# NeuralRevenant/semantic-query-engine

Measured on AMD Instinct MI355X. Metric: k-NN queries/sec (brute-force cosine top-10, 1024-d, 10M vectors), higher is better.
Workload: dtype i8; 1 GPU; flat cosine top-10, N=10000000 x 1024 fp32 (int8 collect scan (per-row-scaled int8 copy, sample-derived thresholds) + fp32 re-score of the candidates, exactness certified per query, bf16 collect pass for uncertified queries), batch=1024 queries/step, index row-sharded over 1 GPU(s); rows=10000000, dim=1024, batch=1024, k=10, parallelism=shard1, scan_mode=int8

## Files before the change

### include/sqe.h

```cpp
#ifndef SQE_H
#define SQE_H

#include <stdint.h>

#ifdef __cplusplus
extern "C" {
#endif

#define SQE_VERSION 100

typedef struct sqe_ctx sqe_ctx;
typedef struct sqe_index sqe_index;
typedef struct sqe_cache sqe_cache;
typedef struct sqe_encoder sqe_encoder;
typedef struct sqe_tokenizer sqe_tokenizer;

enum {
    SQE_OK = 0,
    SQE_ERR_INVALID = -1,
    SQE_ERR_HIP = -2,
    SQE_ERR_OOM = -3,
    SQE_ERR_STATE = -4,
    SQE_ERR_UNSUPPORTED = -5,
    SQE_ERR_IO = -6
// ... 57 lines not shown
int sqe_index_search_collapsed_device(sqe_index* idx, const float* q_dev, int B, int k,
                                      float* cos_out_dev, int64_t* id_out_dev, int64_t* key_out_dev);

int sqe_index_train(sqe_index* idx, const float* x_host, int64_t n, int iters, uint64_t seed);
int sqe_index_train_device(sqe_index* idx, const float* x_dev, int64_t n, int iters, uint64_t seed);
int sqe_index_ivf_export(sqe_index* idx, float* centroids_host, int32_t* assign_host);

typedef struct sqe_i8_launch_t {
    int64_t rows;
    int64_t tile_stride;
    int32_t dim, B, b_pad, k;
    int32_t tile_rows;
    int32_t q_pitch;
    int32_t query_block;
    int32_t n_chunks;
    int32_t list_cap;
    int32_t sample_int8;
    int32_t sample_step;
    int32_t sample_tiles, sample_chunks, sample_b_pad, sample_m;
    int32_t uncertified;
    int32_t pool_cap;
} sqe_i8_launch_t;
enum { SQE_I8_ROWS = 0, SQE_I8_ROW_SCALES = 1, SQE_I8_QUERIES = 2, SQE_I8_THRESHOLDS = 3, SQE_I8_LIST_COUNTS = 4, SQE_I8_LISTS = 5,
       SQE_I8_SAMPLE_BEST = 6, SQE_I8_POOL_COUNTS = 7, SQE_I8_POOLS = 8, SQE_I8_QUERIES_TILED = 9 };
int sqe_index_i8_last(sqe_index* idx, sqe_i8_launch_t* out);
int sqe_index_i8_read(sqe_index* idx, int what, int64_t offset, void* out_host, int64_t bytes);

typedef struct sqe_index_state_t {
    int64_t rows;
    int64_t i8_rows;
    int64_t i8_tile_stride;
    int32_t dim;
    int32_t scan_pitch;
    int32_t last_B;
    int32_t last_i8;
} sqe_index_state_t;
enum { SQE_STATE_SCAN_BF16 = 0, SQE_STATE_RESID_MAX = 1, SQE_STATE_I8_RESID_MAX = 2, SQE_STATE_QN = 3, SQE_STATE_Q_RESID = 4,
       SQE_STATE_Q8_RESID = 5, SQE_STATE_Q8_SCALES = 6 };
int sqe_index_state(sqe_index* idx, sqe_index_state_t* out);
int sqe_index_state_read(sqe_index* idx, int what, int64_t offset, void* out_host, int64_t bytes);

int sqe_index_save(sqe_index* idx, const char* path);
int sqe_index_load(sqe_ctx* ctx, const char* path, sqe_index** out);

int sqe_merge_topk_device(sqe_ctx* ctx, const float* cos_parts_dev, const int64_t* id_parts_dev,
                          int64_t part_stride_bytes, int P, int B, int k,
                          float* cos_out_dev, int64_t* id_out_dev);
// ... 67 lines not shown
```

### semantic_query_engine_amd/csrc/api.hip

```cpp
#include <math.h>
#include <stdio.h>
#include <stdlib.h>
#include <string.h>

#include <algorithm>
#include <memory>
#include <new>
#include <vector>

#include "internal.h"

namespace sqe {

static thread_local std::string g_last_error;

void set_error(const std::string& msg) { g_last_error = msg; }
int fail(int code, const std::string& msg) {
    g_last_error = msg;
    return code;
}

int index_grow(sqe_index* idx, int64_t need_rows, hipStream_t s) {
    if (need_rows <= idx->cap) return SQE_OK;
    const int64_t n = idx->n.load();
// ... 395 lines not shown

int sqe_index_i8_read(sqe_index* idx, int what, int64_t offset, void* out_host, int64_t bytes) {
    if (!idx || (!out_host && bytes > 0)) return fail(SQE_ERR_INVALID, "sqe_index_i8_read: null argument");
    if (idx->group || idx->ivf) return fail(SQE_ERR_UNSUPPORTED, "sqe_index_i8_read: single-device FLAT indexes only");
    OpScope op(idx->ctx, idx->ord, true);
    const sqe_i8_launch_t& L = idx->i8_launch;
    const bool copy_only = what == SQE_I8_ROWS || what == SQE_I8_ROW_SCALES;
    if (L.rows == 0 && !(copy_only && idx->i8db.p && idx->i8_rows > 0))
        return fail(SQE_ERR_STATE, copy_only ? "sqe_index_i8_read: this index has no int8 copy of its rows"
                                             : "sqe_index_i8_read: this index has not answered a search with the int8 first pass");
    const int64_t tiles = L.rows ? (L.rows + L.tile_rows - 1) / L.tile_rows : (idx->i8_rows + SCAN_BM - 1) / SCAN_BM;
    const void* src = nullptr;
    int64_t size = 0;
    switch (what) {
        case SQE_I8_ROWS: src = idx->i8db.p; size = tiles * idx->i8_tile_stride; break;
        case SQE_I8_ROW_SCALES: src = idx->i8sxi.p; size = tiles * SCAN_BM * 4; break;
        case SQE_I8_QUERIES: src = idx->q8.p; size = (int64_t)L.b_pad * L.q_pitch; break;
        case SQE_I8_QUERIES_TILED: src = idx->q8t.p; size = ((int64_t)L.b_pad + 255) / 256 * 256 * L.dim; break;
        case SQE_I8_THRESHOLDS: src = idx->i8thr_int.p; size = (int64_t)L.b_pad * 4; break;
        case SQE_I8_LIST_COUNTS: src = idx->cand_cnt.p; size = (int64_t)L.n_chunks * L.b_pad * 4; break;
        case SQE_I8_LISTS: src = idx->cand.p; size = (int64_t)L.n_chunks * L.b_pad * L.list_cap * 8; break;
        case SQE_I8_POOL_COUNTS: src = idx->i8ovf_cnt.p; size = (int64_t)L.b_pad * 4; break;
        case SQE_I8_POOLS: src = idx->i8ovf.p; size = (int64_t)L.b_pad * L.pool_cap * 8; break;
        case SQE_I8_SAMPLE_BEST:
            if (!L.sample_int8) return fail(SQE_ERR_STATE, "sqe_index_i8_read: the threshold pass of the last search did not run in int8");
            src = idx->i8samp.p; size = (int64_t)L.sample_chunks * L.sample_b_pad * 16 * 8; break;
        default: return fail(SQE_ERR_INVALID, "sqe_index_i8_read: unknown buffer");
    }
    if (offset < 0 || bytes < 0 || offset + bytes > size) return fail(SQE_ERR_INVALID, "sqe_index_i8_read: range outside the buffer");
    if (bytes == 0) return SQE_OK;
    SQE_HIP(hipMemcpyAsync(out_host, static_cast<const char*>(src) + offset, (size_t)bytes, hipMemcpyDeviceToHost, op.s));
    SQE_HIP(hipStreamSynchronize(op.s));
    return SQE_OK;
}

int sqe_index_state(sqe_index* idx, sqe_index_state_t* out) {
    if (!idx || !out) return fail(SQE_ERR_INVALID, "sqe_index_state: null argument");
    if (idx->group || idx->ivf) return fail(SQE_ERR_UNSUPPORTED, "sqe_index_state: single-device FLAT indexes only");
    OpScope op(idx->ctx, idx->ord, true);
    out->rows = idx->n.load();
    out->i8_rows = idx->i8db.p ? idx->i8_rows : 0;
    out->i8_tile_stride = idx->i8db.p ? idx->i8_tile_stride : 0;
    out->dim = idx->dim;
    out->scan_pitch = idx->pitch;
    out->last_B = idx->last_B;
    out->last_i8 = idx->last_i8 ? 1 : 0;
// ... 500 lines not shown
```

### semantic_query_engine_amd/csrc/internal.h

```cpp
#pragma once

#include <atomic>
#include <mutex>
#include <string>
#include <vector>

#include "kernels.h"

namespace sqe {

struct DevBuf {
    void* p = nullptr;
    size_t bytes = 0;
    DevBuf() = default;
    DevBuf(const DevBuf&) = delete;
    DevBuf& operator=(const DevBuf&) = delete;
    ~DevBuf() { release(); }
    void release() {
        if (p) (void)hipFree(p);
        p = nullptr;
        bytes = 0;
    }
    int ensure(size_t need) {
        if (need <= bytes) return SQE_OK;
// ... 145 lines not shown
    sqe::DevBuf resid_max;
    sqe::DevBuf q_resid;
    sqe::DevBuf unc;
    sqe::DevBuf fb_keys, fb_cnt;
    sqe::DevBuf unc_ids, thr_c, qb_c;
    sqe::DevBuf stage_in, stage_out;
    int certify = 1;
    sqe::DevBuf i8db;
    sqe::DevBuf i8sxi;
    sqe::DevBuf i8resid_max;
    int64_t i8_cap_tiles = 0, i8_tile_stride = 0;
    int64_t i8_rows = 0;
    sqe::DevBuf q8t;
    sqe::DevBuf q8, q8sqi, q8resid, i8thr_int, i8thr_eff, i8cos_s, i8ids_s, i8stats, i8samp;
    int64_t i8_min_rows = 1000000;
    int i8_sample_step = 100;
    int i8_sample_m = 20;
    float i8_dx = 0.f;
    bool i8_dx_stale = true;
    bool i8_oom_logged = false;
    int i8_sample_int8 = 1;
    double i8_max_resid = 0.02;
    sqe::DevBuf i8ovf, i8ovf_cnt;
    double i8_anchor_margin = 0.25;
    int i8_key_budget = 6144;
    sqe_i8_launch_t i8_launch{};
    int last_B = 0;
    bool last_i8 = false;
    sqe::IvfState* ivf = nullptr;
    bool internal = false;
    sqe::GroupIndex* group = nullptr;
    std::atomic<int64_t> next_id{0};
    bool has_map = false;
    sqe::DevBuf idmap;
    sqe::FilterState* filter = nullptr;
    int64_t filter_gather_rows = 1 << 20;
    sqe::RangeState* range = nullptr;
    int64_t range_key_budget = 1 << 25;
    bool has_keys = false;
    sqe::DevBuf keys;
    sqe::CollapseState* collapse = nullptr;
    int collapse_depth = 0;
};

struct sqe_cache {
    sqe_ctx* ctx = nullptr;
// ... 123 lines not shown
```

### semantic_query_engine_amd/csrc/scan_i8.hip

```cpp
#include <stdlib.h>

#include <type_traits>

#include "scan_common.h"

namespace sqe {

namespace {

typedef __attribute__((ext_vector_type(4))) int i32x4;

constexpr int HALF_BYTES = 64;
constexpr int LINE_BYTES = 128;
constexpr int OPER_BYTES = 128 * LINE_BYTES;
constexpr int NSTAGE = 4;
constexpr int BNQ = 256;
#ifndef SQE_I8_VARIANT
#define SQE_I8_VARIANT 1
#endif
constexpr int I8V = SQE_I8_VARIANT;
constexpr int NSTA = (I8V & 64) ? 5 : NSTAGE;
constexpr int OFF_B = NSTA * OPER_BYTES;
constexpr int OFF_SCALES = OFF_B + NSTAGE * OPER_BYTES;
constexpr int OFF_CNT = OFF_SCALES + 2 * 1024;
constexpr int OFF_FLAGS = OFF_CNT + BNQ * 4;
constexpr int LDS_BYTES = OFF_FLAGS + 64;
constexpr int BLOCK_BYTES = SCAN_BM * HALF_BYTES;
static_assert(LDS_BYTES <= 160 * 1024, "LDS budget");

struct I8KernelArgs {
    const int8_t* db8;
    long long tile_stride;
    const uint32_t* sxi;
    const int8_t* q8;
    int q_pitch;
    const int8_t* q8t;
    const int* thr_int;
    int64_t n_rows;
    int K, B, b_pad, n_tiles, n_chunks, qblocks;
    uint64_t* cand;
    int* cand_cnt;
    uint64_t* ovf;
    int* ovf_cnt;
    unsigned long long* stamps;
    int dbg;
};

#define I8_BARRIER()                           \
    do {                                       \
        __builtin_amdgcn_sched_barrier(0);     \
        __builtin_amdgcn_s_barrier();          \
        __builtin_amdgcn_sched_barrier(0);     \
    } while (0)
#define I8_WAIT(imm)                               \
    do {                                           \
        __builtin_amdgcn_sched_barrier(0);         \
        __builtin_amdgcn_s_waitcnt(imm);           \
        __builtin_amdgcn_sched_barrier(0);         \
    } while (0)
#define I8_WAIT_VM8_LGKM0() I8_WAIT(0x0078)
#define I8_WAIT_VM7_LGKM0() I8_WAIT(0x0077)
#define I8_WAIT_VM0_LGKM0() I8_WAIT(0x0070)

typedef i32x4 AOps[8];
typedef i32x4 BOps[4];

struct Cur {
    int e, h;
    const char* tile;
};

struct S8 {
    const char* qbase;
    const char* scales_src;
    long long scales_stride = 1024;
    char* smem;
    unsigned offA0, offA1;
    unsigned rdA, rdB;
    int wave, wm, wn, lane;
    int nt, HS, J;
    long long tile_bytes;
    Cur rd, dm;
    int order;
    int pend_h, pend_stage;
    bool defer_on;

    __device__ __forceinline__ void advance(Cur& c) const {
        if (++c.h == HS) {
            c.h = 0;
            ++c.e;
            c.tile += tile_bytes;
        }
    }
    __device__ __forceinline__ void scale_piece(const Cur& c) const {
        lds_dma16_sbase(scales_src + (long long)c.e * scales_stride, (unsigned)lane * 16u, smem + OFF_SCALES + (c.e & 1) * 1024);
    }
    __device__ __forceinline__ void issue_a(const Cur& c, int stage) const {
        char* st = smem + stage * OPER_BYTES;
        const char* as = c.tile + (long long)c.h * BLOCK_BYTES;
        lds_dma16_sbase(as, offA0, st + wave * 1024);
        lds_dma16_sbase(as, offA1, st + (wave + 8) * 1024);
    }
    __device__ __forceinline__ void issue_b(int h, int stage, int which) const {
        char* st = smem + OFF_B + stage * OPER_BYTES;
        const char* bs = qbase + h * BLOCK_BYTES;
        if (which == 0) lds_dma16_sbase(bs, offA0, st + wave * 1024);
        else lds_dma16_sbase(bs, offA1, st + (wave + 8) * 1024);
    }
    __device__ __forceinline__ void issue(const Cur& c, int stage, bool all) const {
        if (wave == 0 && c.h == 0) scale_piece(c);
        issue_a(c, stage);
        issue_b(c.h, stage, 0);
        if (all) issue_b(c.h, stage, 1);
    }
};

template <bool FIRST>
__device__ __forceinline__ void cmp_phase(i32x4 (&acc)[8][4], const AOps& a, const BOps& b) {
#pragma unroll
    for (int fm = 0; fm < 8; ++fm)
#pragma unroll
        for (int fn = 0; fn < 4; ++fn)
            acc[fm][fn] = __builtin_amdgcn_mfma_i32_16x16x64_i8(a[fm], b[fn], FIRST ? i32x4{0, 0, 0, 0} : acc[fm][fn], 0, 0, 0);
}

__device__ __forceinline__ void cmp_phase_mid(S8& P, i32x4 (&acc)[8][4], const AOps& a, const BOps& b) {
#pragma unroll
    for (int fm = 0; fm < 8; ++fm) {
        if (fm == 2) {
            __builtin_amdgcn_sched_barrier(0);
            if (P.pend_h >= 0) {
                P.issue_b(P.pend_h, P.pend_stage, 1);
                P.pend_h = -1;
// ... 151 lines not shown
    if (tid < 16) flags[tid] = 0;
    uint64_t* cand_base = p.cand + ((size_t)chunk * p.b_pad + q0) * CAND_CAP;
    uint64_t* ovf_base = p.ovf + (size_t)q0 * I8_OVF_CAP;
    int* ovf_cnt = p.ovf_cnt + q0;
    const int q_live = min(BNQ, p.B - q0);

    {
        const int line = P.wave * 8 + (lane >> 3);
        const int c = (lane & 7) ^ ((line >> 1) & 7);
        const int row = line + 128 * (c >> 2);
        P.offA0 = (unsigned)(row * HALF_BYTES) + (c & 3) * 16;
        P.offA1 = P.offA0 + (unsigned)(64 * HALF_BYTES);
    }
    {
        const int r = lane & 15, cq = lane >> 4, sw = (r >> 1) & 7;
        P.rdA = (unsigned)(r * LINE_BYTES + (((P.wm * 4 + cq) ^ sw) << 4));
        P.rdB = (unsigned)(((P.wn & 1) * 64 + r) * LINE_BYTES + ((((P.wn >> 1) * 4 + cq) ^ sw) << 4));
    }
    P.qbase = reinterpret_cast<const char*>(p.q8t) + (size_t)qb * P.HS * BLOCK_BYTES;
    P.scales_src = reinterpret_cast<const char*>(p.sxi + (size_t)tile_begin * SCAN_BM);
    const char* tile0 = reinterpret_cast<const char*>(p.db8) + (long long)tile_begin * p.tile_stride;
    P.rd = Cur{0, 0, tile0};
    P.dm = Cur{0, 0, tile0};

    int thr[4];
#pragma unroll
    for (int c = 0; c < 4; ++c) thr[c] = p.thr_int[q0 + P.wn * 64 + c * 16 + (lane & 15)];

    i32x4 acc[8][4];
    AOps a;
    BOps b;

    constexpr bool DEEP = (I8V & 64) != 0;
    int dmb_h = 0;
    int ia = 0, ra = 0;
    if (P.J > 0) {
        for (int s = 0; s < 3 && s < P.J; ++s) {
            P.issue(P.dm, s, true);
            P.advance(P.dm);
        }
        if (DEEP) {
            dmb_h = 3 % P.HS;
            ia = 3;
            if (3 < P.J) {
                P.issue_a(P.dm, 3);
                P.advance(P.dm);
// ... 10 lines not shown
        unsigned cols = 0;
        const bool sync_appends = (p.dbg & 7) == 2;
        int* any_cols = flags + 8;
        int tile_scale = 1;
        auto last_phase = [&](int e) {
            tile_scale = __builtin_amdgcn_readfirstlane(*reinterpret_cast<const int*>(smem + OFF_SCALES + (e & 1) * 1024));
            int tlo[4];
            tile_thresholds(thr, tile_scale, tlo);
            cols = cmp_phase_last(acc, a, b, tlo);
            if (sync_appends && cols != 0 && fresh_lane() == 0) *any_cols = 1;
        };
#ifdef SQE_DEBUG_KNOBS
        const bool dbg_no_store = ((p.dbg >> 3) & 32) != 0;
#else
        constexpr bool dbg_no_store = false;
#endif
        auto tile_end = [&](int e) {
#ifdef SQE_DEBUG_KNOBS
            if (p.stamps && tid == 0 && (blockIdx.x == 0 || blockIdx.x == 100) && ((e & (e - 1)) == 0 || e == P.nt - 1)) {
                const int slot = e == P.nt - 1 ? 31 : (e == 0 ? 0 : 1 + (31 - __builtin_clz(e)));
                unsigned long long* o = p.stamps + (blockIdx.x ? 128 : 0) + slot * 3;
                o[0] = (unsigned long long)e + 1; o[1] = wall_clock64(); o[2] = clock64();
            }
#endif
            if (sync_appends) {
                const bool any = __builtin_amdgcn_readfirstlane(*any_cols) != 0;
                if (!any) return;
            }
            if (cols) {
                const int fl = fresh_lane();
                const int64_t tile_row0 = (int64_t)(tile_begin + e) * SCAN_BM;
                const int64_t row_base = tile_row0 + P.wm * 128 + (fl >> 4) * 4;
                const bool partial = tile_row0 + SCAN_BM > p.n_rows;
                const int qc0 = P.wn * 64 + (fl & 15);
                if (cols & 1u) collect_group<0>(acc, row_base, p.n_rows, partial, qc0, qc0 < q_live, thr[0], tile_scale, cnt, cand_base, ovf_base, ovf_cnt, dbg_no_store);
                if (cols & 2u) collect_group<1>(acc, row_base, p.n_rows, partial, qc0 + 16, qc0 + 16 < q_live, thr[1], tile_scale, cnt, cand_base, ovf_base, ovf_cnt, dbg_no_store);
                if (cols & 4u) collect_group<2>(acc, row_base, p.n_rows, partial, qc0 + 32, qc0 + 32 < q_live, thr[2], tile_scale, cnt, cand_base, ovf_base, ovf_cnt, dbg_no_store);
                if (cols & 8u) collect_group<3>(acc, row_base, p.n_rows, partial, qc0 + 48, qc0 + 48 < q_live, thr[3], tile_scale, cnt, cand_base, ovf_base, ovf_cnt, dbg_no_store);
            }
            __builtin_amdgcn_sched_barrier(0);
            if (sync_appends) {
                I8_BARRIER();
                if (tid == 0) *any_cols = 0;
            }
        };
#ifndef SQE_I8_TWO_BARRIERS
        auto issue_next = [&](int jj) {
            if (DEEP) {
                if (jj + 3 < P.J) {
                    P.issue_b(dmb_h, (jj + 3) & 3, 0);
                    P.issue_b(dmb_h, (jj + 3) & 3, 1);
                    dmb_h = dmb_h + 1 == P.HS ? 0 : dmb_h + 1;
                }
                if (jj + 4 < P.J) {
                    if (P.wave == 0 && P.dm.h == 0) P.scale_piece(P.dm);
                    P.issue_a(P.dm, ia);
                    P.advance(P.dm);
                    ia = ia + 1 == NSTA ? 0 : ia + 1;
                }
                return;
            }
            if (jj + 3 < P.J) {
                P.issue(P.dm, (jj + 3) & 3, true);
                P.advance(P.dm);
            }
        };
        auto wait_pieces = [&](int jj) {
            if (DEEP) {
                if (jj + 4 < P.J) I8_WAIT(0x0F76);
                else if (jj + 3 < P.J) I8_WAIT(0x0F74);
                else I8_WAIT(0x0F70);
                return;
            }
            if (jj + 3 < P.J) I8_WAIT(0x0F74);
            else I8_WAIT(0x0F70);
        };
        auto read_next = [&](int x, bool b_first = false) {
            read_operands(P, a, b, x, DEEP ? ra : (x & 3), b_first);
            if (DEEP) ra = ra + 1 == NSTA ? 0 : ra + 1;
        };
#ifdef SQE_DEBUG_KNOBS
        const int xdbg = p.dbg >> 3;
#define I8_PRIO(n) do { if (!(xdbg & 4)) __builtin_amdgcn_s_setprio(n); } while (0)
#else
        constexpr int xdbg = 0;
#define I8_PRIO(n) __builtin_amdgcn_s_setprio(n)
#endif
        auto g0_head = [&](int jj) {
            if (!(I8V & 3)) issue_next(jj);
        };
        auto g0_tail = [&](int jj) {
            if (I8V & 2) {
                if (jj + 1 < P.J) read_next(jj + 1);
                issue_next(jj);
                wait_pieces(jj);
                return;
            }
            if (I8V & 1) issue_next(jj);
            wait_pieces(jj);
            if (jj + 1 < P.J) read_next(jj + 1);
        };
        auto g1_head = [&](int jj) {
            if (I8V & 8) {
                read_next(jj, (I8V & 128) != 0);
                issue_next(jj);
                return;
            }
            issue_next(jj);
            read_next(jj, (I8V & 128) != 0);
        };
        if (group == 0) {
            read_next(0);
            for (int e = 0; e < P.nt; ++e) {
                g0_head(j);
                I8_PRIO(2);
                cmp_phase<true>(acc, a, b);
                I8_PRIO(0);
                g0_tail(j);
                I8_BARRIER();
                ++j;
                for (int h = 1; h < HS - 1; ++h) {
                    g0_head(j);
                    I8_PRIO(2);
                    cmp_phase<false>(acc, a, b);
                    I8_PRIO(0);
                    g0_tail(j);
                    I8_BARRIER();
                    ++j;
                }
                g0_head(j);
                I8_PRIO(2);
                last_phase(e);
                I8_PRIO(0);
                g0_tail(j);
                if (xdbg & 16) tile_end(e);
                I8_BARRIER();
// ... 10 lines not shown
                I8_BARRIER();
                ++j;
                for (int h = 1; h < HS - 1; ++h) {
                    g1_head(j);
                    I8_PRIO(2);
                    cmp_phase<false>(acc, a, b);
                    I8_PRIO(0);
                    wait_pieces(j);
                    I8_BARRIER();
                    ++j;
                }
                g1_head(j);
                I8_PRIO(2);
                last_phase(e);
                I8_PRIO(0);
                wait_pieces(j);
                if (xdbg & 16) tile_end(e);
                I8_BARRIER();
                ++j;
                if (!(xdbg & 16)) tile_end(e);
            }
        }
#undef I8_PRIO
#else
        if (group == 0) {
            mem_phase(P, a, b, 0, false);
            I8_BARRIER();
            for (int e = 0; e < P.nt; ++e) {
                cmp_phase<true>(acc, a, b);
                I8_BARRIER();
                mem_phase(P, a, b, j + 1, P.defer_on && HS > 2);
                I8_BARRIER();
                ++j;
                for (int h = 1; h < HS - 1; ++h) {
                    cmp_phase_mid(P, acc, a, b);
                    I8_BARRIER();
                    mem_phase(P, a, b, j + 1, P.defer_on && h < HS - 2);
                    I8_BARRIER();
                    ++j;
                }
                last_phase(e);
                I8_BARRIER();
                if (j + 1 < P.J) mem_phase(P, a, b, j + 1, false);
                I8_BARRIER();
                ++j;
                tile_end(e);
// ... 5 lines not shown
                I8_BARRIER();
                cmp_phase<true>(acc, a, b);
                I8_BARRIER();
                ++j;
                for (int h = 1; h < HS - 1; ++h) {
                    mem_phase(P, a, b, j, P.defer_on);
                    I8_BARRIER();
                    cmp_phase_mid(P, acc, a, b);
                    I8_BARRIER();
                    ++j;
                }
                mem_phase(P, a, b, j, false);
                I8_BARRIER();
                last_phase(e);
                I8_BARRIER();
                ++j;
                tile_end(e);
            }
        }
#endif
    }
    asm volatile("s_waitcnt vmcnt(0)" ::: "memory");
    __syncthreads();
    for (int i = tid; i < BNQ; i += SCAN_THREADS) p.cand_cnt[(size_t)chunk * p.b_pad + q0 + i] = cnt[i];
}

struct I8SampleKernelArgs {
    const int8_t* db8; long long tile_stride; const uint32_t* sxi;
    const int8_t* q8t;
    int K, b_pad, n_tiles_s, step, n_chunks, qblocks;
    int2* out;
};

__global__ __launch_bounds__(SCAN_THREADS) void sample_i8_pp_kernel(I8SampleKernelArgs p) {
    extern __shared__ __attribute__((aligned(16))) char smem[];
    const int tid = threadIdx.x;
    const int lane = tid & 63;
    S8 P;
    P.lane = lane;
    P.wave = __builtin_amdgcn_readfirstlane(tid >> 6);
    const int group = P.wave >> 2;
    P.wm = P.wave >> 2;
    P.wn = P.wave & 3;
    P.order = 0;
    P.pend_h = -1;
    P.pend_stage = 0;
// ... 445 lines not shown
int launch_stream(const I8KernelArgs& k, hipStream_t stream) {
    const int lds = BN * (k.K + 128) + BN * 4 + SCAN_NWAVES * 192 * 9;
    auto kern = scan_i8_stream_kernel<BN, RING>;
    SQE_HIP(ensure_dynamic_lds(reinterpret_cast<const void*>(kern), lds));
    hipLaunchKernelGGL(kern, dim3(k.n_chunks * k.qblocks), dim3(SCAN_THREADS), lds, stream, k);
    SQE_HIP(hipGetLastError());
    return SQE_OK;
}

template <int WM, int WN, int FM, int FN, int NST, int NSTB>
int launch_small(const I8KernelArgs& k, hipStream_t stream) {
    constexpr int BN = WN * FN * 16;
    constexpr int LDS = (NST * SCAN_BM + NSTB * BN) * 128 + 2048 + BN * 4;
    static_assert(LDS <= 160 * 1024, "LDS budget");
    auto kern = scan_i8_small_kernel<WM, WN, FM, FN, NST, NSTB>;
    SQE_HIP(ensure_dynamic_lds(reinterpret_cast<const void*>(kern), LDS));
    hipLaunchKernelGGL(kern, dim3(k.n_chunks * k.qblocks), dim3(SCAN_THREADS), LDS, stream, k);
    SQE_HIP(hipGetLastError());
    return SQE_OK;
}

}

int launch_scan_i8(const I8ScanArgs& a, hipStream_t stream) {
    if (a.K % 128 != 0 || a.K < 256) return fail(SQE_ERR_INVALID, "int8 scan: dim must be a multiple of 128, >= 256");
    if (a.bn != 64 && a.bn != 128 && a.bn != BNQ) return fail(SQE_ERR_INVALID, "int8 scan: query block must be 64, 128 or 256");
    if (a.qblocks * a.bn != a.b_pad) return fail(SQE_ERR_INVALID, "int8 scan: padded batch must be a whole number of query blocks");
    I8KernelArgs k;
    k.db8 = a.db8; k.tile_stride = a.tile_stride; k.sxi = a.sxi; k.q8 = a.q8; k.q_pitch = a.q_pitch; k.q8t = a.q8t; k.thr_int = a.thr_int;
    k.n_rows = a.n_rows; k.K = a.K; k.B = a.B; k.b_pad = a.b_pad; k.n_tiles = a.n_tiles; k.n_chunks = a.n_chunks; k.qblocks = a.qblocks;
    k.cand = a.cand; k.cand_cnt = a.cand_cnt; k.ovf = a.ovf; k.ovf_cnt = a.ovf_cnt; k.stamps = a.stamps;
    if (!a.ovf || !a.ovf_cnt) return fail(SQE_ERR_INVALID, "int8 scan: no overflow pool");
    {
        static const int force = [] { const char* e = knob_env("SQE_I8_SYNC"); return e ? (e[0] == '0' ? 1 : 2) : 0; }();
        static const int xdbg = [] { const char* e = knob_env("SQE_I8_DBG"); return e ? atoi(e) : 0; }();
        k.dbg = force | (xdbg << 3);
    }
    {
        static const bool staged = [] { const char* e = knob_env("SQE_I8_STAGED"); return e && e[0] == '1'; }();
        const int lds = a.bn * (a.K + 128) + a.bn * 4 + SCAN_NWAVES * 192 * 9;
        if (!staged && a.bn <= 128 && lds <= 160 * 1024) {
            if (a.bn == 64 && a.K % 1024 == 0) return launch_stream<64, 32>(k, stream);
            if (a.bn == 64 && a.K % 512 == 0) return launch_stream<64, 16>(k, stream);
            if (a.bn == 128 && a.K % 512 == 0) return launch_stream<128, 16>(k, stream);
        }
    }
    if (a.bn == 64) return launch_small<8, 1, 2, 4, 3, 3>(k, stream);
    if (a.bn == 128) return launch_small<4, 2, 4, 4, 3, 2>(k, stream);
    if (!a.q8t) return fail(SQE_ERR_INVALID, "int8 scan: no tiled query copy");
    auto kern = scan_i8_pp_kernel;
    SQE_HIP(ensure_dynamic_lds(reinterpret_cast<const void*>(kern), LDS_BYTES));
    hipLaunchKernelGGL(kern, dim3(a.n_chunks * a.qblocks), dim3(SCAN_THREADS), LDS_BYTES, stream, k);
    SQE_HIP(hipGetLastError());
    return SQE_OK;
}

int launch_sample_i8(const I8SampleArgs& a, hipStream_t stream) {
    if (a.K % 128 != 0 || a.K < 256) return fail(SQE_ERR_INVALID, "int8 sample: dim must be a multiple of 128, >= 256");
    if (a.b_pad % BNQ != 0 || a.n_tiles_s < 1 || a.step < 1 || a.n_chunks < 1 || a.n_chunks > a.n_tiles_s)
// ... 15 lines not shown
```

### semantic_query_engine_amd/csrc/scan_i8_deep.hip

```cpp
#define SQE_I8_VARIANT 65
#define scan_i8_pp_kernel scan_i8_pp_deep_kernel
#define sample_i8_pp_kernel sample_i8_pp_deep_kernel
#define scan_i8_small_kernel scan_i8_small_deep_kernel
#define launch_scan_i8 launch_scan_i8_deep
#define launch_sample_i8 launch_sample_i8_deep
#include "scan_i8.hip"
```

### semantic_query_engine_amd/csrc/search.hip

```cpp
#include <stdio.h>
#include <stdlib.h>
#include <string.h>

#include <algorithm>
#include <tuple>
#include <utility>

#include "internal.h"

namespace sqe {

__global__ void add_count_kernel(int* acc, const int* v) { *acc += *v; }

namespace {

int auto_kp(const sqe_index* idx, int k) {
    if (idx->rescore_k > 0) return std::min(MAX_KP, std::max(idx->rescore_k, k));
    if (idx->certify) return k <= 32 ? 64 : k <= 128 ? 128 : k;
    return std::min(MAX_KP, std::max(32, 4 * k));
}

struct Pass {
    sqe_index* idx;
    hipStream_t s;
    int64_t n_rows;
    int B, k, kp;
    ScanPlan plan;
    float* cos_out;
    int64_t* id_out;
    int pass_index;
    bool certify;
    int* unc_count;
    float* collect_thr;
    int step8, m8;
};

bool i8_stamps_wanted() {
    static const bool want_stamps = [] { const char* e = knob_env("SQE_I8_STAMPS"); return e && e[0] == '1'; }();
    return want_stamps;
}

bool scan_counters_wanted() {
    static const bool want = [] { const char* e = knob_env("SQE_DBG"); return e && (atoi(e) & 32); }();
    return want;
}

int arm_dbg(sqe_index* idx, hipStream_t s, unsigned long long** slot) {
    SQE_TRY(idx->dbg.ensure(8192));
    SQE_HIP(hipMemsetAsync(idx->dbg.p, 0, 8192, s));
    *slot = idx->dbg.as<unsigned long long>();
    return SQE_OK;
}

int report_i8_stamps(sqe_index* idx, hipStream_t s) {
    unsigned long long h[256];
    SQE_HIP(hipMemcpyAsync(h, idx->dbg.p, sizeof(h), hipMemcpyDeviceToHost, s));
    SQE_HIP(hipStreamSynchronize(s));
    int wall_khz = 0;
    (void)hipDeviceGetAttribute(&wall_khz, hipDeviceAttributeWallClockRate, idx->ctx->device);
    for (int blk = 0; blk < 2; ++blk) {
        const unsigned long long* o = h + blk * 128;
        int prev = -1;
        for (int sl = 0; sl < 32; ++sl) {
            if (!o[sl * 3]) continue;
            if (prev >= 0 && o[sl * 3] > o[prev * 3]) {
                const double tiles = (double)(o[sl * 3] - o[prev * 3]);
                const double us = (double)(o[sl * 3 + 1] - o[prev * 3 + 1]) / (wall_khz / 1e3);
                const double cyc = (double)(o[sl * 3 + 2] - o[prev * 3 + 2]);
                fprintf(stderr, "[sqe i8 stamps] wg %3d tiles %5llu..%5llu: %7.2f us per tile, %7.0f core cycles per tile, %5.0f MHz\n",
                        blk ? 100 : 0, o[prev * 3], o[sl * 3], us / tiles, cyc / tiles, us > 0 ? cyc / us : 0.0);
            }
            prev = sl;
        }
    }
    idx->dbg.release();
    return SQE_OK;
}

int report_scan_counters(const Pass& p) {
    sqe_index* idx = p.idx;
    const ScanPlan& plan = p.plan;
    hipStream_t s = p.s;
    if (!idx->dbg.p) return SQE_OK;
    unsigned long long h[1024];
    SQE_HIP(hipMemcpyAsync(h, idx->dbg.p, 8192, hipMemcpyDeviceToHost, s));
    SQE_HIP(hipStreamSynchronize(s));
    int wall_khz = 0;
    (void)hipDeviceGetAttribute(&wall_khz, hipDeviceAttributeWallClockRate, idx->ctx->device);
    fprintf(stderr, "[sqe dbg] appends=%llu slow_path_entries=%llu compactions=%llu block0_core_ticks=%llu wall_ticks=%llu core_mhz=%.0f\n",
            h[0], h[1], h[2], h[4], h[5], h[5] ? (double)h[4] / (double)h[5] * wall_khz / 1e3 : 0.0);
    for (int blk = 0; blk < 2; ++blk)
        for (int w = 0; w < 8; ++w) {
            const unsigned long long* o = h + 8 + blk * 64 + w * 8;
            if (!o[0]) continue;
            const double n = (double)o[0];
            fprintf(stderr, "[sqe dbg] wg %d wave %d: phases=%llu  cmp %.0f  barrier after cmp %.0f | mem: dma issue %.0f  lds reads issue %.0f  waitcnt %.0f  barrier after mem %.0f\n",
// ... 253 lines not shown
        sa.master = idx->master; sa.qn = idx->qn.as<float>(); sa.K = K; sa.B = B; sa.k = m8;
        sa.cos_out = idx->i8cos_s.as<float>(); sa.id_out = idx->i8ids_s.as<int64_t>();
        SQE_TRY(launch_select_rescore(sa, s));
        SQE_TRY(launch_i8_thresholds(idx->i8cos_s.as<float>(), m8, idx->q8sqi.as<uint32_t>(), K, B, plan.b_pad,
                                     idx->i8thr_int.as<int>(), idx->i8thr_eff.as<float>(), s));
    }
    return SQE_OK;
}

int i8_scan_select(const Pass& p, int q8_pitch) {
    sqe_index* idx = p.idx;
    sqe_ctx* c = idx->ctx;
    const ScanPlan& plan = p.plan;
    hipStream_t s = p.s;
    const int K = idx->dim, B = p.B;
    {
        StageTimer t(c->prof, s, ST_SCAN);
        I8ScanArgs ia;
        ia.db8 = idx->i8db.as<int8_t>(); ia.tile_stride = idx->i8_tile_stride; ia.sxi = idx->i8sxi.as<uint32_t>();
        ia.q8 = idx->q8.as<int8_t>(); ia.q_pitch = q8_pitch; ia.q8t = idx->q8t.as<int8_t>(); ia.thr_int = idx->i8thr_int.as<int>();
        ia.n_rows = p.n_rows; ia.K = K; ia.B = B; ia.b_pad = plan.b_pad; ia.n_tiles = plan.n_tiles; ia.n_chunks = plan.n_chunks;
        ia.qblocks = plan.qblocks; ia.bn = plan.bn; ia.cand = idx->cand.as<uint64_t>(); ia.cand_cnt = idx->cand_cnt.as<int>();
        ia.ovf = idx->i8ovf.as<uint64_t>(); ia.ovf_cnt = idx->i8ovf_cnt.as<int>();
        if (i8_stamps_wanted()) SQE_TRY(arm_dbg(idx, s, &ia.stamps));
        static const int deep_max = [] { const char* e = knob_env("SQE_I8_DEEP_MAX"); return e ? atoi(e) : 1; }();
        if (plan.bn == 256 && plan.qblocks <= deep_max) SQE_TRY(launch_scan_i8_deep(ia, s));
        else SQE_TRY(launch_scan_i8(ia, s));
        if (i8_stamps_wanted()) SQE_TRY(report_i8_stamps(idx, s));
    }
    {
        StageTimer t(c->prof, s, ST_SELECT);
        I8SelectArgs sa;
        sa.cand = idx->cand.as<uint64_t>(); sa.cand_cnt = idx->cand_cnt.as<int>(); sa.n_chunks = plan.n_chunks; sa.b_pad = plan.b_pad;
        sa.master = idx->master; sa.qn = idx->qn.as<float>(); sa.K = K; sa.B = B; sa.k = p.k;
        sa.scan16 = idx->scan; sa.pitch16 = idx->pitch;
        sa.sxi = idx->i8sxi.as<uint32_t>(); sa.sqi = idx->q8sqi.as<uint32_t>();
        sa.q_resid8 = idx->q8resid.as<float>(); sa.db_resid8_max = idx->i8resid_max.as<uint32_t>();
        sa.q_resid16 = idx->q_resid.as<float>(); sa.db_resid16_max = idx->resid_max.as<uint32_t>();
        sa.thr_eff = idx->i8thr_eff.as<float>();
        sa.sample_cos = idx->i8cos_s.as<float>(); sa.sample_ids = idx->i8ids_s.as<int64_t>(); sa.sample_m = p.m8;
        sa.cos_out = p.cos_out; sa.id_out = p.id_out; sa.id_base = search_id_base(idx);
        sa.unc_count = p.unc_count; sa.collect_thr = p.collect_thr;
        sa.stats = idx->i8stats.as<unsigned long long>();
        sa.ovf = idx->i8ovf.as<uint64_t>(); sa.ovf_cnt = idx->i8ovf_cnt.as<int>();
        SQE_TRY(launch_select_i8(sa, s));
    }
    return SQE_OK;
}

int i8_first_pass(const Pass& p) {
    sqe_index* idx = p.idx;
    sqe_ctx* c = idx->ctx;
    const ScanPlan& plan = p.plan;
    hipStream_t s = p.s;
    const int K = idx->dim, B = p.B, step8 = p.step8, m8 = p.m8;
    const int q8_pitch = K + 128;
    const int b_pad_s = (B + 255) / 256 * 256;
    const int b_pad_q = std::max(plan.b_pad, b_pad_s);
    const int64_t full_tiles = p.n_rows / SCAN_BM;
    const int n_tiles_i8s = (int)(full_tiles / step8);
    const bool sample_i8 = idx->i8_sample_int8 != 0 && n_tiles_i8s >= 1;
    SQE_TRY(idx->q8.ensure((size_t)b_pad_q * q8_pitch));
    const size_t q8t_block = (size_t)256 * K;
    const size_t q8t_blocks = ((size_t)b_pad_q + 255) / 256;
    SQE_TRY(idx->q8t.ensure(q8t_blocks * q8t_block));
    SQE_TRY(idx->q8sqi.ensure((size_t)b_pad_q * 4));
    SQE_TRY(idx->q8resid.ensure((size_t)plan.b_pad * 4));
    SQE_TRY(idx->i8thr_int.ensure((size_t)plan.b_pad * 4));
    SQE_TRY(idx->i8thr_eff.ensure((size_t)plan.b_pad * 4));
    SQE_TRY(idx->i8cos_s.ensure((size_t)B * m8 * 4));
    SQE_TRY(idx->i8ids_s.ensure((size_t)B * m8 * 8));
    SQE_TRY(idx->i8stats.ensure(64));
    SQE_TRY(idx->i8ovf.ensure((size_t)plan.b_pad * I8_OVF_CAP * 8));
    SQE_TRY(idx->i8ovf_cnt.ensure((size_t)plan.b_pad * 4));
    {
        StageTimer t(c->prof, s, ST_PREP);
        SQE_HIP(hipMemsetAsync(idx->i8ovf_cnt.p, 0, (size_t)plan.b_pad * 4, s));
        if (b_pad_q > B)
            SQE_HIP(hipMemsetAsync(idx->q8.as<char>() + (size_t)B * q8_pitch, 0, (size_t)(b_pad_q - B) * q8_pitch, s));
        if (B % 256 != 0)
            SQE_HIP(hipMemsetAsync(idx->q8t.as<char>() + (size_t)(B / 256) * q8t_block, 0, (q8t_blocks - (size_t)(B / 256)) * q8t_block, s));
        SQE_TRY(launch_quantize_queries_i8(idx->qn.as<float>(), B, K, idx->q8.as<int8_t>(), q8_pitch, idx->q8t.as<int8_t>(),
                                           idx->q8sqi.as<uint32_t>(), idx->q8resid.as<float>(), s));
        SQE_HIP(hipMemsetAsync(idx->i8stats.p, 0, 64, s));
    }
    int chunks_s_used = 0;
    SQE_TRY(i8_threshold_pass(p, b_pad_s, n_tiles_i8s, sample_i8, &chunks_s_used));
    SQE_TRY(i8_scan_select(p, q8_pitch));
    SQE_TRY(run_collect_fallback(p));
    {
        sqe_i8_launch_t& L = idx->i8_launch;
        L.rows = p.n_rows; L.tile_stride = idx->i8_tile_stride; L.dim = K; L.B = B; L.b_pad = plan.b_pad; L.k = p.k;
        L.tile_rows = SCAN_BM; L.q_pitch = q8_pitch; L.query_block = plan.bn; L.n_chunks = plan.n_chunks; L.list_cap = CAND_CAP; L.pool_cap = I8_OVF_CAP;
        L.sample_int8 = sample_i8 ? 1 : 0; L.sample_step = step8; L.sample_tiles = n_tiles_i8s;
        L.sample_chunks = chunks_s_used;
        L.sample_b_pad = b_pad_s; L.sample_m = m8; L.uncertified = -1;
    }
    SQE_HIP(hipMemcpyAsync(c->i8_last.p, idx->i8stats.p, 32, hipMemcpyDeviceToDevice, s));
    c->i8_valid.store(true);
    return SQE_OK;
// ... 96 lines not shown
```

### semantic_query_engine_amd/engine.py

```python
from __future__ import annotations

import ctypes as C
import threading
import weakref
from typing import Optional, Tuple

import numpy as np

from . import _native as N

INDEX_FLAT = 0
INDEX_IVF_FLAT = 1
SCAN_BF16_RESCORE = 0
SCAN_INT8_RESCORE = 2
KEY_NONE = -(1 << 63)
I8_ROWS, I8_ROW_SCALES, I8_QUERIES, I8_THRESHOLDS, I8_LIST_COUNTS, I8_LISTS, I8_SAMPLE_BEST, I8_POOL_COUNTS, I8_POOLS = range(9)
I8_QUERIES_TILED = 9

STATE_SCAN_BF16, STATE_RESID_MAX, STATE_I8_RESID_MAX, STATE_QN, STATE_Q_RESID, STATE_Q8_RESID, STATE_Q8_SCALES = range(7)


def _f32(a: np.ndarray) -> np.ndarray:
    return np.ascontiguousarray(a, dtype=np.float32)


EXCHANGE_AUTO, EXCHANGE_RCCL, EXCHANGE_COPY = 0, 1, 2


class Context:

    def __init__(self, device: int = 0, devices=None, exchange: int = EXCHANGE_AUTO):
        self.lib = N.load()
        h = C.c_void_p()
        if devices is None:
            ids = (C.c_int32 * 1)(device)
            N.check(self.lib.sqe_create(ids, 1, C.byref(h)))
            self.devices = [device]
        else:
            self.devices = [int(d) for d in devices]
            ids = (C.c_int32 * len(self.devices))(*self.devices)
# ... 335 lines not shown
```

Baseline: 110,700 queries/s.

## Pace int8 scan workgroups sharing a chunk so they stay in lockstep

```diff
diff --git a/include/sqe.h b/include/sqe.h
--- a/include/sqe.h
+++ b/include/sqe.h
@@ -103,7 +103,7 @@
     int32_t pool_cap;
 } sqe_i8_launch_t;
 enum { SQE_I8_ROWS = 0, SQE_I8_ROW_SCALES = 1, SQE_I8_QUERIES = 2, SQE_I8_THRESHOLDS = 3, SQE_I8_LIST_COUNTS = 4, SQE_I8_LISTS = 5,
-       SQE_I8_SAMPLE_BEST = 6, SQE_I8_POOL_COUNTS = 7, SQE_I8_POOLS = 8, SQE_I8_QUERIES_TILED = 9 };
+       SQE_I8_SAMPLE_BEST = 6, SQE_I8_POOL_COUNTS = 7, SQE_I8_POOLS = 8, SQE_I8_QUERIES_TILED = 9, SQE_I8_PROGRESS = 10 };
 int sqe_index_i8_last(sqe_index* idx, sqe_i8_launch_t* out);
 int sqe_index_i8_read(sqe_index* idx, int what, int64_t offset, void* out_host, int64_t bytes);
 
diff --git a/semantic_query_engine_amd/csrc/api.hip b/semantic_query_engine_amd/csrc/api.hip
--- a/semantic_query_engine_amd/csrc/api.hip
+++ b/semantic_query_engine_amd/csrc/api.hip
@@ -441,6 +441,7 @@
         case SQE_I8_LISTS: src = idx->cand.p; size = (int64_t)L.n_chunks * L.b_pad * L.list_cap * 8; break;
         case SQE_I8_POOL_COUNTS: src = idx->i8ovf_cnt.p; size = (int64_t)L.b_pad * 4; break;
         case SQE_I8_POOLS: src = idx->i8ovf.p; size = (int64_t)L.b_pad * L.pool_cap * 8; break;
+        case SQE_I8_PROGRESS: src = idx->i8ovf_cnt.as<int>() + L.b_pad; size = (int64_t)idx->i8_pace_live * 4; break;
         case SQE_I8_SAMPLE_BEST:
             if (!L.sample_int8) return fail(SQE_ERR_STATE, "sqe_index_i8_read: the threshold pass of the last search did not run in int8");
             src = idx->i8samp.p; size = (int64_t)L.sample_chunks * L.sample_b_pad * 16 * 8; break;
diff --git a/semantic_query_engine_amd/csrc/internal.h b/semantic_query_engine_amd/csrc/internal.h
--- a/semantic_query_engine_amd/csrc/internal.h
+++ b/semantic_query_engine_amd/csrc/internal.h
@@ -191,6 +191,7 @@
     int i8_sample_int8 = 1;
     double i8_max_resid = 0.02;
     sqe::DevBuf i8ovf, i8ovf_cnt;
+    int i8_pace_live = 0;
     double i8_anchor_margin = 0.25;
     int i8_key_budget = 6144;
     sqe_i8_launch_t i8_launch{};
diff --git a/semantic_query_engine_amd/csrc/scan_i8.h b/semantic_query_engine_amd/csrc/scan_i8.h
--- /dev/null
+++ b/semantic_query_engine_amd/csrc/scan_i8.h
@@ -0,0 +1,18 @@
+#pragma once
+
+#include "kernels.h"
+
+namespace sqe {
+
+constexpr int PACE_PAD = 16;
+
+inline bool scan_i8_paced(const I8ScanArgs& a) {
+    const int grid = a.n_chunks * a.qblocks;
+    return a.bn == 256 && a.qblocks > 1 && a.qblocks <= PACE_PAD && (grid & 7) == 0 && (grid >> 3) % a.qblocks == 0;
+}
+inline size_t scan_i8_pace_words(const I8ScanArgs& a) { return scan_i8_paced(a) ? (size_t)a.n_chunks * a.qblocks + PACE_PAD : 0; }
+
+int launch_scan_i8_paced(const I8ScanArgs& args, int* pace, hipStream_t stream);
+int launch_scan_i8_deep_paced(const I8ScanArgs& args, int* pace, hipStream_t stream);
+
+}
diff --git a/semantic_query_engine_amd/csrc/scan_i8.hip b/semantic_query_engine_amd/csrc/scan_i8.hip
--- a/semantic_query_engine_amd/csrc/scan_i8.hip
+++ b/semantic_query_engine_amd/csrc/scan_i8.hip
@@ -3,6 +3,7 @@
 #include <type_traits>
 
 #include "scan_common.h"
+#include "scan_i8.h"
 
 namespace sqe {
 
@@ -24,7 +25,11 @@
 constexpr int OFF_SCALES = OFF_B + NSTAGE * OPER_BYTES;
 constexpr int OFF_CNT = OFF_SCALES + 2 * 1024;
 constexpr int OFF_FLAGS = OFF_CNT + BNQ * 4;
-constexpr int LDS_BYTES = OFF_FLAGS + 64;
+constexpr int OFF_PACE = OFF_FLAGS + 64;
+constexpr int LDS_BYTES = OFF_PACE + 2 * 256;
+constexpr int PACE_LAG = 1;
+constexpr int PACE_NAP = 6;
+constexpr int PACE_DONE = 0x7fffffff;
 constexpr int BLOCK_BYTES = SCAN_BM * HALF_BYTES;
 static_assert(LDS_BYTES <= 160 * 1024, "LDS budget");
 
@@ -44,6 +49,8 @@
     int* ovf_cnt;
     unsigned long long* stamps;
     int dbg;
+    int* pace;
+    int pace_lag, pace_nap;
 };
 
 #define I8_BARRIER()                           \
@@ -62,6 +69,11 @@
 #define I8_WAIT_VM7_LGKM0() I8_WAIT(0x0077)
 #define I8_WAIT_VM0_LGKM0() I8_WAIT(0x0070)
 
+__device__ __forceinline__ void lds_dma4_sbase_sc1(const char* uniform_base, unsigned lane_off, char* lds_wave_base) {
+    const unsigned dst = (unsigned)(uintptr_t)(__attribute__((address_space(3))) char*)lds_wave_base;
+    asm volatile("s_mov_b32 m0, %2\n\ts_nop 0\n\tglobal_load_lds_dword %0, %1 sc1" ::"v"(lane_off), "s"(uniform_base), "s"(dst) : "memory");
+}
+
 typedef i32x4 AOps[8];
 typedef i32x4 BOps[4];
 
@@ -74,6 +86,7 @@
     const char* qbase;
     const char* scales_src;
     long long scales_stride = 1024;
+    const char* pace_src = nullptr;
     char* smem;
     unsigned offA0, offA1;
     unsigned rdA, rdB;
@@ -95,6 +108,13 @@
     __device__ __forceinline__ void scale_piece(const Cur& c) const {
         lds_dma16_sbase(scales_src + (long long)c.e * scales_stride, (unsigned)lane * 16u, smem + OFF_SCALES + (c.e & 1) * 1024);
     }
+    __device__ __forceinline__ void pace_piece(const Cur& c) const {
+        lds_dma4_sbase_sc1(pace_src, (unsigned)(lane & (PACE_PAD - 1)) * 4u, smem + OFF_PACE + (c.e & 1) * 256);
+    }
+    __device__ __forceinline__ void tile_pieces(const Cur& c) const {
+        scale_piece(c);
+        if (pace_src) pace_piece(c);
+    }
     __device__ __forceinline__ void issue_a(const Cur& c, int stage) const {
         char* st = smem + stage * OPER_BYTES;
         const char* as = c.tile + (long long)c.h * BLOCK_BYTES;
@@ -108,7 +128,7 @@
         else lds_dma16_sbase(bs, offA1, st + (wave + 8) * 1024);
     }
     __device__ __forceinline__ void issue(const Cur& c, int stage, bool all) const {
-        if (wave == 0 && c.h == 0) scale_piece(c);
+        if (wave == 0 && c.h == 0) tile_pieces(c);
         issue_a(c, stage);
         issue_b(c.h, stage, 0);
         if (all) issue_b(c.h, stage, 1);
@@ -306,6 +326,8 @@
     const char* tile0 = reinterpret_cast<const char*>(p.db8) + (long long)tile_begin * p.tile_stride;
     P.rd = Cur{0, 0, tile0};
     P.dm = Cur{0, 0, tile0};
+    int* const pace_mine = p.pace ? p.pace + (size_t)chunk * p.qblocks + qb : nullptr;
+    if (p.pace) P.pace_src = reinterpret_cast<const char*>(p.pace + (size_t)chunk * p.qblocks);
 
     int thr[4];
 #pragma unroll
@@ -362,7 +384,10 @@
                 unsigned long long* o = p.stamps + (blockIdx.x ? 128 : 0) + slot * 3;
                 o[0] = (unsigned long long)e + 1; o[1] = wall_clock64(); o[2] = clock64();
             }
+            if (p.stamps && tid == 0 && blockIdx.x < 256 && (e == min(100, P.nt / 4) || e == min(400, 3 * P.nt / 4)))
+                p.stamps[512 + blockIdx.x * 2 + (e == min(100, P.nt / 4) ? 0 : 1)] = wall_clock64();
 #endif
+            if (pace_mine && tid == 0) __hip_atomic_store(pace_mine, e + 1, __ATOMIC_RELAXED, __HIP_MEMORY_SCOPE_AGENT);
             if (sync_appends) {
                 const bool any = __builtin_amdgcn_readfirstlane(*any_cols) != 0;
                 if (!any) return;
@@ -393,7 +418,7 @@
                     dmb_h = dmb_h + 1 == P.HS ? 0 : dmb_h + 1;
                 }
                 if (jj + 4 < P.J) {
-                    if (P.wave == 0 && P.dm.h == 0) P.scale_piece(P.dm);
+                    if (P.wave == 0 && P.dm.h == 0) P.tile_pieces(P.dm);
                     P.issue_a(P.dm, ia);
                     P.advance(P.dm);
                     ia = ia + 1 == NSTA ? 0 : ia + 1;
@@ -429,6 +454,26 @@
         auto g0_head = [&](int jj) {
             if (!(I8V & 3)) issue_next(jj);
         };
+#ifdef SQE_DEBUG_KNOBS
+        const int pace_lag = p.pace_lag > 0 ? p.pace_lag : PACE_LAG;
+        unsigned naps = 0;
+#else
+        constexpr int pace_lag = PACE_LAG;
+#endif
+        auto pace_nap = [&](int e) {
+            const int v = *reinterpret_cast<const int*>(smem + OFF_PACE + (e & 1) * 256 + lane * 4);
+            const bool behind = lane < p.qblocks && lane != qb && v != 0 && e - 1 - v >= pace_lag;
+            if (!__any(behind)) return;
+#ifdef SQE_DEBUG_KNOBS
+            ++naps;
+            if (p.pace_nap > 0) {
+                for (int i = 0; i < p.pace_nap; ++i) __builtin_amdgcn_s_sleep(32);
+                return;
+            }
+#endif
+#pragma unroll
+            for (int i = 0; i < PACE_NAP; ++i) __builtin_amdgcn_s_sleep(32);
+        };
         auto g0_tail = [&](int jj) {
             if (I8V & 2) {
                 if (jj + 1 < P.J) read_next(jj + 1);
@@ -452,6 +497,7 @@
         if (group == 0) {
             read_next(0);
             for (int e = 0; e < P.nt; ++e) {
+                if (pace_mine && P.wave == 0) pace_nap(e);
                 g0_head(j);
                 I8_PRIO(2);
                 cmp_phase<true>(acc, a, b);
@@ -508,6 +554,9 @@
             }
         }
 #undef I8_PRIO
+#ifdef SQE_DEBUG_KNOBS
+        if (p.stamps && naps && tid == 0) atomicAdd(p.stamps + 300, (unsigned long long)naps);
+#endif
 #else
         if (group == 0) {
             mem_phase(P, a, b, 0, false);
@@ -559,6 +608,7 @@
     }
     asm volatile("s_waitcnt vmcnt(0)" ::: "memory");
     __syncthreads();
+    if (pace_mine && tid == 0) __hip_atomic_store(pace_mine, PACE_DONE, __ATOMIC_RELAXED, __HIP_MEMORY_SCOPE_AGENT);
     for (int i = tid; i < BNQ; i += SCAN_THREADS) p.cand_cnt[(size_t)chunk * p.b_pad + q0 + i] = cnt[i];
 }
 
@@ -1050,7 +1100,9 @@
 
 }
 
-int launch_scan_i8(const I8ScanArgs& a, hipStream_t stream) {
+int launch_scan_i8(const I8ScanArgs& a, hipStream_t stream) { return launch_scan_i8_paced(a, nullptr, stream); }
+
+int launch_scan_i8_paced(const I8ScanArgs& a, int* pace, hipStream_t stream) {
     if (a.K % 128 != 0 || a.K < 256) return fail(SQE_ERR_INVALID, "int8 scan: dim must be a multiple of 128, >= 256");
     if (a.bn != 64 && a.bn != 128 && a.bn != BNQ) return fail(SQE_ERR_INVALID, "int8 scan: query block must be 64, 128 or 256");
     if (a.qblocks * a.bn != a.b_pad) return fail(SQE_ERR_INVALID, "int8 scan: padded batch must be a whole number of query blocks");
@@ -1063,6 +1115,16 @@
         static const int force = [] { const char* e = knob_env("SQE_I8_SYNC"); return e ? (e[0] == '0' ? 1 : 2) : 0; }();
         static const int xdbg = [] { const char* e = knob_env("SQE_I8_DBG"); return e ? atoi(e) : 0; }();
         k.dbg = force | (xdbg << 3);
+    }
+    k.pace = scan_i8_paced(a) ? pace : nullptr;
+    k.pace_lag = k.pace_nap = 0;
+    if (k.pace) {
+        const char* on = knob_env("SQE_I8_PACE");
+        const char* lag = knob_env("SQE_I8_PACE_LAG");
+        const char* nap = knob_env("SQE_I8_PACE_NAP");
+        if (on && on[0] == '0') k.pace = nullptr;
+        if (lag) k.pace_lag = atoi(lag);
+        if (nap) k.pace_nap = atoi(nap);
     }
     {
         static const bool staged = [] { const char* e = knob_env("SQE_I8_STAGED"); return e && e[0] == '1'; }();
diff --git a/semantic_query_engine_amd/csrc/scan_i8_deep.hip b/semantic_query_engine_amd/csrc/scan_i8_deep.hip
--- a/semantic_query_engine_amd/csrc/scan_i8_deep.hip
+++ b/semantic_query_engine_amd/csrc/scan_i8_deep.hip
@@ -3,5 +3,6 @@
 #define sample_i8_pp_kernel sample_i8_pp_deep_kernel
 #define scan_i8_small_kernel scan_i8_small_deep_kernel
 #define launch_scan_i8 launch_scan_i8_deep
+#define launch_scan_i8_paced launch_scan_i8_deep_paced
 #define launch_sample_i8 launch_sample_i8_deep
 #include "scan_i8.hip"
diff --git a/semantic_query_engine_amd/csrc/search.hip b/semantic_query_engine_amd/csrc/search.hip
--- a/semantic_query_engine_amd/csrc/search.hip
+++ b/semantic_query_engine_amd/csrc/search.hip
@@ -7,6 +7,7 @@
 #include <utility>
 
 #include "internal.h"
+#include "scan_i8.h"
 
 namespace sqe {
 
@@ -36,8 +37,8 @@
 };
 
 bool i8_stamps_wanted() {
-    static const bool want_stamps = [] { const char* e = knob_env("SQE_I8_STAMPS"); return e && e[0] == '1'; }();
-    return want_stamps;
+    const char* e = knob_env("SQE_I8_STAMPS");
+    return e && e[0] == '1';
 }
 
 bool scan_counters_wanted() {
@@ -52,8 +53,8 @@
     return SQE_OK;
 }
 
-int report_i8_stamps(sqe_index* idx, hipStream_t s) {
-    unsigned long long h[256];
+int report_i8_stamps(sqe_index* idx, hipStream_t s, const ScanPlan& plan) {
+    static unsigned long long h[1024];
     SQE_HIP(hipMemcpyAsync(h, idx->dbg.p, sizeof(h), hipMemcpyDeviceToHost, s));
     SQE_HIP(hipStreamSynchronize(s));
     int wall_khz = 0;
@@ -72,6 +73,36 @@
             }
             prev = sl;
         }
+    }
+    const int G = plan.n_chunks * plan.qblocks;
+    if (plan.qblocks > 1 && G <= 256 && wall_khz > 0) {
+        const int nt = plan.n_tiles / plan.n_chunks;
+        const int at[2] = {std::min(100, nt / 4), std::min(400, 3 * nt / 4)};
+        double tile_us = 0;
+        int n_us = 0;
+        for (int blk = 0; blk < G; ++blk)
+            if (h[512 + blk * 2] && h[512 + blk * 2 + 1] > h[512 + blk * 2] && at[1] > at[0]) {
+                tile_us += (double)(h[512 + blk * 2 + 1] - h[512 + blk * 2]) / (wall_khz / 1e3) / (at[1] - at[0]);
+                ++n_us;
+            }
+        tile_us = n_us ? tile_us / n_us : 1.0;
+        double worst[2] = {0, 0}, mean[2] = {0, 0};
+        int over[2] = {0, 0};
+        for (int c = 0; c < plan.n_chunks; ++c)
+            for (int t = 0; t < 2; ++t) {
+                unsigned long long lo = ~0ull, hi = 0;
+                for (int qb = 0; qb < plan.qblocks; ++qb) {
+                    const int logical = c * plan.qblocks + qb;
+                    const int blk = (G & 7) == 0 ? (logical % (G >> 3)) * 8 + logical / (G >> 3) : logical;
+                    const unsigned long long v = h[512 + blk * 2 + t];
+                    lo = std::min(lo, v); hi = std::max(hi, v);
+                }
+                const double d = (double)(hi - lo) / (wall_khz / 1e3) / tile_us;
+                worst[t] = std::max(worst[t], d); mean[t] += d / plan.n_chunks; over[t] += d >= 1.0;
+            }
+        fprintf(stderr, "[sqe i8 stamps] spread between the %d workgroups of a chunk when they finish tile %d / %d, in tiles (one tile = %.1f us): "
+                        "mean %.2f / %.2f, worst %.2f / %.2f, a tile or more in %d / %d of %d chunks; naps taken %llu\n",
+                plan.qblocks, at[0], at[1], tile_us, mean[0], mean[1], worst[0], worst[1], over[0], over[1], plan.n_chunks, h[300]);
     }
     idx->dbg.release();
     return SQE_OK;
@@ -371,11 +402,13 @@
         ia.n_rows = p.n_rows; ia.K = K; ia.B = B; ia.b_pad = plan.b_pad; ia.n_tiles = plan.n_tiles; ia.n_chunks = plan.n_chunks;
         ia.qblocks = plan.qblocks; ia.bn = plan.bn; ia.cand = idx->cand.as<uint64_t>(); ia.cand_cnt = idx->cand_cnt.as<int>();
         ia.ovf = idx->i8ovf.as<uint64_t>(); ia.ovf_cnt = idx->i8ovf_cnt.as<int>();
+        int* pace = idx->i8_pace_live ? ia.ovf_cnt + plan.b_pad : nullptr;
         if (i8_stamps_wanted()) SQE_TRY(arm_dbg(idx, s, &ia.stamps));
-        static const int deep_max = [] { const char* e = knob_env("SQE_I8_DEEP_MAX"); return e ? atoi(e) : 1; }();
-        if (plan.bn == 256 && plan.qblocks <= deep_max) SQE_TRY(launch_scan_i8_deep(ia, s));
-        else SQE_TRY(launch_scan_i8(ia, s));
-        if (i8_stamps_wanted()) SQE_TRY(report_i8_stamps(idx, s));
+        int deep_max = 1;
+        if (const char* e = knob_env("SQE_I8_DEEP_MAX")) deep_max = atoi(e);
+        if (plan.bn == 256 && plan.qblocks <= deep_max) SQE_TRY(launch_scan_i8_deep_paced(ia, pace, s));
+        else SQE_TRY(launch_scan_i8_paced(ia, pace, s));
+        if (i8_stamps_wanted()) SQE_TRY(report_i8_stamps(idx, s, plan));
     }
     {
         StageTimer t(c->prof, s, ST_SELECT);
@@ -421,10 +454,14 @@
     SQE_TRY(idx->i8ids_s.ensure((size_t)B * m8 * 8));
     SQE_TRY(idx->i8stats.ensure(64));
     SQE_TRY(idx->i8ovf.ensure((size_t)plan.b_pad * I8_OVF_CAP * 8));
-    SQE_TRY(idx->i8ovf_cnt.ensure((size_t)plan.b_pad * 4));
+    I8ScanArgs shape;
+    shape.bn = plan.bn; shape.n_chunks = plan.n_chunks; shape.qblocks = plan.qblocks;
+    const size_t pace_words = scan_i8_pace_words(shape);
+    idx->i8_pace_live = pace_words ? plan.n_chunks * plan.qblocks : 0;
+    SQE_TRY(idx->i8ovf_cnt.ensure(((size_t)plan.b_pad + pace_words) * 4));
     {
         StageTimer t(c->prof, s, ST_PREP);
-        SQE_HIP(hipMemsetAsync(idx->i8ovf_cnt.p, 0, (size_t)plan.b_pad * 4, s));
+        SQE_HIP(hipMemsetAsync(idx->i8ovf_cnt.p, 0, ((size_t)plan.b_pad + pace_words) * 4, s));
         if (b_pad_q > B)
             SQE_HIP(hipMemsetAsync(idx->q8.as<char>() + (size_t)B * q8_pitch, 0, (size_t)(b_pad_q - B) * q8_pitch, s));
         if (B % 256 != 0)
diff --git a/semantic_query_engine_amd/engine.py b/semantic_query_engine_amd/engine.py
--- a/semantic_query_engine_amd/engine.py
+++ b/semantic_query_engine_amd/engine.py
@@ -16,6 +16,7 @@
 KEY_NONE = -(1 << 63)
 I8_ROWS, I8_ROW_SCALES, I8_QUERIES, I8_THRESHOLDS, I8_LIST_COUNTS, I8_LISTS, I8_SAMPLE_BEST, I8_POOL_COUNTS, I8_POOLS = range(9)
 I8_QUERIES_TILED = 9
+I8_PROGRESS = 10
 
 STATE_SCAN_BF16, STATE_RESID_MAX, STATE_I8_RESID_MAX, STATE_QN, STATE_Q_RESID, STATE_Q8_RESID, STATE_Q8_SCALES = range(7)
 
```

Result: no change. 109,900 queries/s (-0.7%).
